# nickmass/mass-raytrace

Measured on AMD Instinct MI355X. Metric: Msamples/sec (rays traced/sec) at 1920×1080×1024spp; 1/2/4/8-GPU scaling, higher is better.
Workload: dtype f32

## Files before the change

mass-raytrace_amd/csrc/device/layout.h:

```cpp
#pragma once
#include <stdint.h>

#include "nf_bound.h"

namespace mrt {

enum : uint32_t { KIND_BOX = 1, KIND_SPHERE = 2, KIND_TRI = 3, KIND_INST = 4, KIND_MODEL = 5, KIND_VOLUME = 6 };
constexpr uint32_t kBoxFlag = 0x80000000u;
constexpr uint32_t kLdsTag = 0x40000000u;
constexpr uint32_t kIdxMask = 0x3FFFFFFFu;
constexpr uint32_t KIND_END = 0;
enum : uint32_t { TRI_FLAG_ALPHA = 1u, TRI_FLAG_UV = 2u, TRI_FLAG_EVE = 4u };
constexpr uint32_t kTriAlpha = 0x80000000u;
constexpr uint32_t kTriIdMask = 0x0FFFFFFFu;

constexpr uint32_t kNfIdx = 0x0FFFFFFFu;
constexpr uint32_t kNfForceL = 0x10000000u, kNfForceR = 0x20000000u;
constexpr uint32_t kNfPop = 0x0FFFFFFFu;
constexpr int kNfExpMin = -100;
constexpr uint32_t kNfStack = 24u;
constexpr uint32_t kNfWildFew = 16u;
constexpr uint32_t kNoParent = 0xFFFFFFFFu;
constexpr uint32_t kWorldKey = 0x80000000u;
enum : uint32_t { VNF_SPHERE = 0, VNF_TRI = 1, VNF_INST = 2, VNF_MODEL = 3 };

constexpr uint32_t SURF_PROGRAM = 0xFFu;
constexpr uint32_t kSurfStack = 4;
struct GpuSurfOp {
  uint32_t op, tex, arg, pad;
  float color[4];
};
struct GpuSurfRef {
  uint32_t kind, index, len, pad;
  float color[4];
};

struct GpuMaterial {
  uint32_t kind, surf_kind, texture;
  float param;
  float color[4];
  uint32_t left, right;
  uint32_t surf_len;
  uint32_t pad1;
// ... 23 lines not shown
  const uint32_t* sph_mat;
  const float* tri_shade;
  const GpuMaterial* materials;
  const GpuTexture* textures;
  const uint32_t* texels;
  uint32_t fast_ok;
  uint32_t n_slots, n_tris, n_sph, n_inst, n_models, n_materials, n_textures, n_texels;
  uint32_t* dbg;
  const float* vol_nid;
  const uint32_t* vol_mat;
  const float* ln_table;
  uint32_t n_vol;
  const GpuSurfOp* surf_ops;
  uint32_t n_surf_ops;
  uint32_t bg_kind;
  float bg_color[4];
  const GpuSurfRef* bg_faces;
  const float* bg_m;
  const uint32_t* slots_tl;
  const uint32_t* tlet;
  uint32_t n_tlet;
  uint32_t tl_world_begin;
  uint32_t nf_ok, nf_world;
  const uint32_t* vnf_leaf;
  uint32_t vnf_base[4];
  uint32_t n_vnf;
  NfBound nfb;
  const float* eve;
  const float* tri_tb;
  uint32_t n_eve;
};

}
```

mass-raytrace_amd/csrc/device/nf_tree.cpp:

```cpp
#include <math.h>
#include <cmath>
#include <string.h>

#include <algorithm>
#include <unordered_map>

#include "upload.h"

namespace mrt {

namespace {

float u2f(uint32_t u) {
  float f;
  memcpy(&f, &u, 4);
  return f;
}
uint32_t f2u(float f) {
  uint32_t u;
  memcpy(&u, &f, 4);
  return u;
}

uint32_t kind_of(const std::vector<uint32_t>& w, uint32_t i) { return w[4 * (i + 1) + 3]; }
// ... 593 lines not shown
    if (!ref_order(s.world_begin, true, world_objs)) return true;
    if (world_objs.empty()) return (s.nf_note = "an empty world", true);
    std::vector<std::vector<uint32_t>> blas_objs(s.blas_regions.size());
    if (s.keep_nf_boxes) {
      s.nf_leaf_box.assign(3 * s.vnf_leaf.size(), NAN);
      s.nf_inst_wild.assign(d.n_instances, 0);
    }
    for (size_t k = 0; k < s.blas_regions.size(); ++k) {
      region_of[s.blas_regions[k].begin] = k;
      if (!ref_order(s.blas_regions[k].begin, false, blas_objs[k])) return true;
    }
    std::vector<uint8_t> by_model(s.blas_regions.size(), 0), by_inst(s.blas_regions.size(), 0);
    for (uint32_t r : world_objs) {
      const uint32_t kd = kind_of(w, r);
      if (kd != KIND_INST && kd != KIND_MODEL) continue;
      auto it = region_of.find(w[4 * (size_t)r + 1]);
      if (it != region_of.end()) (kd == KIND_MODEL ? by_model : by_inst)[it->second] = 1;
    }
    const uint32_t has_blas = s.blas_regions.empty() ? 0 : 2;
    std::vector<Tree> blas(s.blas_regions.size());
    blas_box.assign(s.blas_regions.size(), Box{});
    blas_bound.assign(s.blas_regions.size(), TriBound{});
    uint32_t blas_depth = 0;
    const uint32_t world_min = Tree::min_levels((uint32_t)world_objs.size());
    if (world_min + has_blas > kNfStack) return (s.nf_note = "too many world objects for the walk's stack", true);
    for (size_t k = 0; k < blas.size(); ++k) {
      for (uint32_t r : blas_objs[k]) {
        blas[k].items.push_back({object_box(r, &blas_bound[k]), r});
        keep_box(r, blas[k].items.back().b);
      }
      if (blas[k].items.empty()) continue;
      blas[k].max_depth = kNfStack - 2 - world_min;
      blas[k].build(0, (uint32_t)blas[k].items.size(), 0);
      blas_depth = std::max(blas_depth, blas[k].depth);
      blas_box[k] = blas[k].nodes[0].b;
      if (by_model[k]) grow_bound(world_tri, blas_bound[k]);
    }
    Tree world;
    NfBound& B = s.nfb;
    B = NfBound{};
    double aw0 = 0, aw1 = 0, bw0 = 0, bw1 = 0, ko1 = 0, ao0 = 0, ao1 = 0, orad = 0;
    std::vector<Item> wild_items, items;
    Box gen_box;
    uint32_t n_world_inst = 0;
    for (uint32_t r : world_objs) n_world_inst += kind_of(w, r) == KIND_INST;
    const bool few = n_world_inst <= kNfWildFew;
    for (uint32_t r : world_objs) {
// ... 21 lines not shown
        ko1 = std::max(ko1, m.ko);
        if (it != region_of.end()) {
          const Box& bb = blas_box[it->second];
          for (int c = 0; c < 8; ++c) {
            const double x = c & 1 ? bb.mx[0] : bb.mn[0], y = c & 2 ? bb.mx[1] : bb.mn[1], z = c & 4 ? bb.mx[2] : bb.mn[2];
            orad = std::max(orad, std::sqrt(x * x + y * y + z * z));
          }
          ao0 = std::max(ao0, ob.a0), ao1 = std::max(ao1, ob.a1);
        }
        if (wild(m) || (few && m.b0 > 0x1p-14)) {
          wild_items.push_back({b, r, true});
          wild_term[r] = {b, m};
          s.nf_wild++;
          if (s.keep_nf_boxes) s.nf_inst_wild[w[4 * (size_t)r]] = 1;
          continue;
        }
        aw0 = std::max(aw0, m.w0), aw1 = std::max(aw1, m.w1), bw0 = std::max(bw0, m.b0), bw1 = std::max(bw1, m.b1);
      }
      if (generic) gen_box.grow(b);
      items.push_back({b, r});
    }
    aw0 = std::max(aw0, world_tri.a0), aw1 = std::max(aw1, world_tri.a1);
    if (r_min < 0x1p-60) return (s.nf_note = "a sphere too small for the walk's rounding bound", true);
    world.items = items;
    world.items.insert(world.items.end(), wild_items.begin(), wild_items.end());
    world.max_depth = kNfStack - (has_blas ? 2 + blas_depth : 0);
    world.build(0, (uint32_t)world.items.size(), 0);
    if (!wild_items.empty()) world.mark_forced(0);
    if (aw1 > 0 || ao1 > 0)
      for (Tree* t : [&] {
             std::vector<Tree*> v{&world};
             for (Tree& b : blas) v.push_back(&b);
             return v;
           }())
        fit_cones(*t);
    s.nf_stack_need = world.depth + (has_blas ? 2 + blas_depth : 0);
    if (s.nf_stack_need > kNfStack) return (s.nf_note = "trees deeper than the walk's stack", true);
    auto ball = [](const Box& b, float c[3], float& rr) {
      double r2 = 0;
      for (int k = 0; k < 3; ++k) {
        const double m = 0.5 * ((double)b.mn[k] + (double)b.mx[k]);
        c[k] = (float)m;
        const double e = std::max(std::fabs((double)b.mx[k] - c[k]), std::fabs(c[k] - (double)b.mn[k]));
        r2 += e * e;
      }
      rr = f_up(std::sqrt(r2) * (1 + 0x1p-40));
    };
    Box wb;
    for (const Item& it : items) wb.grow(it.b);
    if (items.empty()) wb = world.nodes[0].b;
    for (int k = 0; k < 3; ++k)
      if (!(std::fabs(wb.mn[k]) < INFINITY && std::fabs(wb.mx[k]) < INFINITY))
        return (s.nf_note = "a box the node format cannot hold (not finite)", true);
    ball(wb, B.wc, B.wr);
    if (aw1 > 0) ball(gen_box, B.gc, B.gr);
    B.aw0 = f_up(aw0), B.aw1 = f_up(aw1), B.bw0 = f_up(bw0 + 0x1p-90), B.bw1 = f_up(bw1);
    B.kw1 = f_up(world_tri.k1), B.ko1 = f_up(ko1);
    B.ao0 = f_up(ao0), B.ao1 = f_up(ao1), B.orad = f_up(orad);
    B.kmax = kNfKappaMax;
    B.kc = (aw1 > 0 || ao1 > 0) ? f_up(1.0001 * 24.0 * kU * 64.0 / (1.0 - 1.01 * (double)kNfKappaMax) * (1.0 + 0x1p-17))
                                : 0.0f;
    B.kcmin = 0.0f;
    if (!gen_extent.empty()) {
      std::nth_element(gen_extent.begin(), gen_extent.begin() + gen_extent.size() / 2, gen_extent.end());
      B.kcmin = std::ldexp(gen_extent[gen_extent.size() / 2], -6);
    }
    if (r_max > 0) {
      ball(sph_box, B.sc, B.sr);
      B.s51 = f_up(51.2 * kU / r_min), B.s28 = f_up(27.8 * kU), B.s130 = f_up(130.2 * kU), B.s11 = f_up(11.2 * kU * r_max);
    } else {
      B.sr = -1.0f;
    }
    s.nf_world = emit(world);
    if (s.nf_world == ~0u) return (s.nf_note = "a box the node format cannot hold (not finite)", true);
    for (size_t k = 0; k < blas.size(); ++k) {
      if (blas[k].items.empty()) continue;
      const uint32_t root = emit(blas[k]);
      if (root == ~0u) return (s.nf_note = "a box the node format cannot hold (not finite)", true);
      blas_root[s.blas_regions[k].begin] = root;
    }
    for (auto& [at, r] : wild_at) {
      const auto& [b, m] = wild_term.at(r);
      bool finite = true;
      for (int k = 0; k < 3; ++k) finite = finite && std::fabs(b.mn[k]) < INFINITY && std::fabs(b.mx[k]) < INFINITY;
      if (!finite) continue;
      float c[3], rr;
      ball(b, c, rr);
      const uint32_t e = push(f2u(b.mn[0]), f2u(b.mn[1]), f2u(b.mn[2]), f2u(b.mx[0]));
      push(f2u(b.mx[1]), f2u(b.mx[2]), f2u(f_up(m.w0)), f2u(f_up(m.w1)));
      push(f2u(f_up(m.b0 + 0x1p-90)), f2u(f_up(m.b1)), f2u(c[0]), f2u(c[1]));
      push(f2u(c[2]), f2u(rr), 0, 0);
      w[4 * (size_t)at + 3] = e;
    }
    for (auto& [rec, ref_blas] : patches) {
      auto it = blas_root.find(ref_blas);
      if (it == blas_root.end()) return (s.nf_note = "an instance of an empty BLAS", true);
      w[4 * rec + 1] = it->second;
    }
    if (n_slots() > kNfIdx) return (s.nf_note = "record stream past 2^28 slots", true);
    s.nf_ok = true;
    return true;
  }
};

}

bool build_nf_trees(const mrt_scene_desc& d, HostScene& s, std::string& err) {
  Builder b{d, s, err, s.slots, {}, {}};
  const size_t keep = s.slots.size();
  const bool ok = b.run();
  if (!s.nf_ok) {
    s.slots.resize(keep);
    s.nf_boxes = 0;
    s.nf_wild = 0;
    s.nf_cones = 0;
    s.vnf_leaf.clear();
  }
  return ok;
}

}
```

mass-raytrace_amd/csrc/device/trace.hip:

```cpp
#include <string.h>

#include <algorithm>

#include "ctx.h"

using namespace mrt;

namespace {

constexpr size_t kTraceLdsMaxBytes = 160 * 1024;
constexpr uint32_t kStashQuads = 4;

template <bool COUNT, bool LDS, uint32_t ALPHA, bool RNG, int BLK, bool NF = false>
__global__ __launch_bounds__(BLK) __attribute__((amdgpu_waves_per_eu(NF ? (COUNT ? 1 : 5) : (ALPHA == 0 && !RNG && !COUNT ? 8 : 1)))) void k_trace(DevScene S, PathBufs in, uint4* hits, Ctrl* ctrl, uint32_t cur,
                                                  DevCounters* cnt, float tmin, float tmax, TraceTune tune) {
  static_assert(!NF || (!LDS && !RNG), "the near-first walk has no treelet and no traversal draws");
  constexpr int R = 1;
  const uint32_t n = ctrl->active[cur];
  if (blockIdx.x == 0 && threadIdx.x == 0) {
    ctrl->active[cur ^ 1] = 0;
    ctrl->surv[cur ^ 1] = 0;
  }
  if (n == 0) return;
  if (LDS) {
    for (uint32_t k = threadIdx.x; k < S.n_tlet; k += BLK) mrt_lds[k] = reinterpret_cast<const uint4*>(S.tlet)[k];
    __syncthreads();
  }
  TravIn tin_{S, reinterpret_cast<const uint4*>(LDS ? S.slots_tl : S.slots), LDS ? S.tl_world_begin : S.world_begin,
              in.ro, in.rd, tmin, in.rng, tmax};
  if (!LDS && !NF) {
    tin_.stash = reinterpret_cast<float4*>(mrt_lds) + threadIdx.x;
    tin_.stash_stride = (uint32_t)BLK;
  }
  const TravIn& tin = tin_;
  const NfStack stk{reinterpret_cast<uint32_t*>(mrt_lds) + threadIdx.x, (uint32_t)BLK};
  LocalCounters lc;
  uint32_t seg = 0, nh = 0;
  uint32_t pool = 0, pool_end = 0;
  bool drained = false;
// ... 15 lines not shown
    }
    if (n_idle >= tune.refill * R || n_idle == 64u * R) {
      while (pool == pool_end && !drained) {
        const uint32_t lo = (uint32_t)((uint64_t)n * grp / kGroups), hi = (uint32_t)((uint64_t)n * (grp + 1) / kGroups);
        uint32_t b = 0;
        if (lane_id() == 0) b = atomicAdd(&ctrl->group_next[grp * 32], tune.chunk);
        b = __shfl(b, 0, 64);
        if (b < hi - lo) {
          pool = lo + b;
          pool_end = hi - pool > tune.chunk ? pool + tune.chunk : hi;
        } else if (++visited == kGroups) {
          drained = true;
        } else {
          grp = (grp + 1) % kGroups;
        }
      }
      const uint32_t avail = pool_end - pool;
      uint32_t off = 0;
      unsigned long long live = 0;
#pragma unroll
      for (int q = 0; q < R; ++q) {
        if (t[q].ray == kIdle) {
          const uint32_t r = off + lane_rank(idle[q]);
          if (r < avail) trav_init<RNG, LDS>(tin, t[q], MRT_IDX(S, pool + r, n, 20), tmax, NF ? S.nf_world : 0xFFFFFFFFu);
        }
        off += (uint32_t)__popcll(idle[q]);
        live |= __ballot(t[q].ray != kIdle);
      }
      pool += n_idle < avail ? n_idle : avail;
      if (live == 0) break;
    }
#pragma unroll
    for (int q = 0; q < R; ++q) {
      auto box_step = [&]() {
        const bool run_box = trav_at_box(t[q]);
        const unsigned long long bm = __builtin_amdgcn_ballot_w64(run_box);
        if ((uint32_t)__popcll(bm) < tune.box_min) return false;
        if (run_box) {
          if (NF && t[q].sp != kExactMode)
            trav_box_index_nf<COUNT>(tin, stk, t[q], lc);
          else
            trav_box_index<COUNT>(tin, t[q], lc);
        }
        if (run_box && (!NF || t[q].sp != kNfDone)) trav_fetch<LDS>(tin, t[q]);
        if (COUNT) {
          lc.wave_slots += lane_id() == 0 ? 64u : 0u;
          lc.lane_steps += run_box ? 1u : 0u;
        }
        return true;
      };
      while (box_step() && box_step()) {
      }
      for (;;) {
        const bool busy = !t[q].done && (!NF || t[q].sp != kNfDone);
        const bool at_box = busy && trav_at_box(t[q]);
        const unsigned long long box_mask = __ballot(at_box);
        const unsigned long long prim_mask = __ballot(busy && !at_box);
        const bool prim_run = NF && (uint32_t)__popcll(prim_mask) >= tune.prim_run;
        const bool box_go = at_box && !prim_run;
        const bool prim_go = (__popcll(prim_mask) >= tune.prim_batch || box_mask == 0) && busy && !at_box;
        if (box_go) {
          if (NF && t[q].sp != kExactMode)
            trav_box_index_nf<COUNT>(tin, stk, t[q], lc);
          else
            trav_box_index<COUNT>(tin, t[q], lc);
        }
        if (prim_go) {
          if (NF && t[q].sp != kExactMode)
            trav_prim_index_nf<COUNT, ALPHA>(tin, stk, t[q], lc);
          else
            trav_prim_index<COUNT, ALPHA, RNG, LDS>(tin, t[q], lc);
        }
        if ((box_go || prim_go) && !t[q].done && (!NF || t[q].sp != kNfDone)) trav_fetch<LDS>(tin, t[q]);
        if (COUNT) {
          lc.wave_slots += lane_id() == 0 ? 64u : 0u;
          lc.lane_steps += (box_go || prim_go) ? 1u : 0u;
        }
        if (!prim_run) break;
      }
      if (NF) {
        const bool over = t[q].sp == kNfDone;
        const unsigned long long om = __builtin_amdgcn_ballot_w64(over);
        if (om != 0 && ((uint32_t)__popcll(om) >= tune.nf_batch ||
                        __builtin_amdgcn_ballot_w64(!t[q].done && !over) == 0) && over) {
          nf_finish<COUNT>(tin, t[q], lc);
          if (!t[q].done) trav_fetch<LDS>(tin, t[q]);
        }
      }
    }
#pragma unroll
    for (int q = 0; q < R; ++q) {
      if (t[q].ray != kIdle && t[q].done) {
        if (RNG) trav_store_rng(tin, t[q]);
        const Hit h = trav_hit<LDS>(tin, t[q]);
        hits[t[q].ray] = make_uint4(__float_as_uint(h.t), h.prim, h.container, 0u);
        seg += 1;
        nh += t[q].prim != kRefNone;
        t[q].ray = kIdle;
      }
    }
  }
  if (COUNT) flush_counters(cnt, lc, seg, nh, 0, 0);
}
// ... 39 lines not shown
template <bool EXT>
__global__ __launch_bounds__(kBlock) void k_rays_out(DevScene S, PathBufs in, const uint4* hits, uint32_t n,
                                                     uint4* out) {
  uint32_t i = blockIdx.x * kBlock + threadIdx.x;
  if (i >= n) return;
  const float4 o4 = in.ro[i], d4 = in.rd[i];
  const uint4 hv = hits[i];
  Hit h{__uint_as_float(hv.x), hv.y, hv.z};
  uint32_t front = 0;
  LocalCounters lc;
  if (h.prim != kRefNone)
    front = resolve_hit<EXT>(S, V3{o4.x, o4.y, o4.z}, V3{d4.x, d4.y, d4.z}, h, lc).front_face ? 1u : 0u;
  out[i] = make_uint4(h.prim, h.container, __float_as_uint(h.prim != kRefNone ? h.t : 0.0f), front);
}

using TraceFn = void (*)(DevScene, PathBufs, uint4*, Ctrl*, uint32_t, DevCounters*, float, float, TraceTune);
template <bool COUNT, uint32_t ALPHA, bool RNG>
TraceFn trace_kernel_lds(int block) {
  return block == 1024  ? k_trace<COUNT, true, ALPHA, RNG, 1024>
         : block == 512 ? k_trace<COUNT, true, ALPHA, RNG, 512>
                        : k_trace<COUNT, true, ALPHA, RNG, kBlock>;
}
template <bool COUNT, uint32_t ALPHA>
TraceFn trace_kernel_a(bool lds, bool rng, int block, bool nf) {
  if (nf) return k_trace<COUNT, false, ALPHA, false, kBlock, true>;
  if (lds) return rng ? trace_kernel_lds<COUNT, ALPHA, true>(block) : trace_kernel_lds<COUNT, ALPHA, false>(block);
  return rng ? k_trace<COUNT, false, ALPHA, true, kBlock> : k_trace<COUNT, false, ALPHA, false, kBlock>;
}
template <bool COUNT>
TraceFn trace_kernel_c(bool lds, uint32_t alpha, bool rng, int block, bool nf) {
  return alpha == 2   ? trace_kernel_a<COUNT, 2>(lds, rng, block, nf)
         : alpha == 1 ? trace_kernel_a<COUNT, 1>(lds, rng, block, nf)
                      : trace_kernel_a<COUNT, 0>(lds, rng, block, nf);
}
TraceFn trace_kernel(bool count, bool lds, uint32_t alpha, bool rng, int block, bool nf) {
  return count ? trace_kernel_c<true>(lds, alpha, rng, block, nf) : trace_kernel_c<false>(lds, alpha, rng, block, nf);
}

}

uint32_t persistent_grid(mrt_ctx* c, const void* f, size_t smem, bool shared, int block, int share_num,
                         int share_den) {
  auto key = std::make_pair(f, smem);
  auto it = c->grids.find(key);
  if (it != c->grids.end()) return it->second;
  if (smem > 0) HIP_CHECK(hipFuncSetAttribute(f, hipFuncAttributeMaxDynamicSharedMemorySize, (int)kTraceLdsMaxBytes));
  int per_cu = 0;
  HIP_CHECK(hipOccupancyMaxActiveBlocksPerMultiprocessor(&per_cu, f, block, smem));
  if (shared) per_cu = std::max(1, per_cu * share_num / share_den);
  if (c->tun.wgs_per_cu) per_cu = (int)c->tun.wgs_per_cu;
  const uint32_t g = (uint32_t)c->cus * (uint32_t)std::max(1, per_cu);
  c->grids[key] = g;
  return g;
}

void launch_trace(mrt_ctx* c, hipStream_t st, const Queue& q, const PathBufs& in, uint32_t cur, bool count,
                  float tmin, float tmax) {
  const Tuning& t = c->tun;
  const bool nf = t.use_nf, lds = !nf && c->facts.treelet;
  const uint32_t alpha = c->scene_alpha ? (c->scene_ext ? 2u : 1u) : 0u;
  const int block = lds ? t.trace_block : kBlock;
  const TraceFn f = trace_kernel(count, lds, alpha, c->facts.trav_rng, block, nf);
  const size_t smem = nf ? (size_t)kNfStack * block * 4 : lds ? (size_t)c->S.n_tlet * 16 : (size_t)kStashQuads * block * 16;
  uint32_t grid = persistent_grid(c, (const void*)f, smem, t.queues > 1, block, nf ? 1 : 3, nf ? 1 : 4);
  const uint32_t nf_cap = 3u * (uint32_t)c->cus;
  if (nf && t.queues > 1 && !t.wgs_per_cu && grid > nf_cap) grid = c->grids[std::make_pair((const void*)f, smem)] = nf_cap;
  hipLaunchKernelGGL(f, dim3(grid), dim3(block), smem, st, c->S, in, q.hits, q.ctrl, cur, c->d_cnt, tmin, tmax, t.trace);
  HIP_CHECK(hipGetLastError());
}

void launch_trace_simple(mrt_ctx* c, const Queue& q, uint32_t cur) {
  auto* f = c->facts.trav_rng ? k_trace_simple<true> : k_trace_simple<false>;
  hipLaunchKernelGGL(f, dim3(c->trace_grid), dim3(kBlock), 0, q.stream, c->S, q.bufs[cur], q.hits, q.ctrl, cur, c->d_cnt);
  HIP_CHECK(hipGetLastError());
}

extern "C" int mrt_trace_rays(mrt_ctx* c, const float* rays, uint32_t n, float t_min, float t_max, mrt_hit* out) {
  MRT_DEV0(c, mrt_trace_rays(c, rays, n, t_min, t_max, out));
  return guarded(c, [&] {
    if (!c->has_scene) throw ApiError{MRT_ERR_STATE, "no scene uploaded"};
    if (n == 0) return;
    if (!rays || !out) throw ApiError{MRT_ERR_INVALID, "null argument"};
    if (n > c->rays_cap) {
      hipFree(c->d_rays);
      hipFree(c->d_rhits);
      c->d_rays = nullptr;
// ... 30 lines not shown
```

mass-raytrace_amd/csrc/device/upload.h:

```cpp
#pragma once
#include <string>
#include <vector>

#include "../../../include/massrt.h"
#include "layout.h"

namespace mrt {

struct BlasRegion {
  uint32_t begin, end, refs;
  bool model;
};

struct HostScene {
  std::vector<uint32_t> slots;
  std::vector<uint32_t> rec_starts;
  uint32_t world_begin = 0, world_end = 0;
  std::vector<float> inst_inv, inst_fwd;
  std::vector<uint32_t> inst_mat, model_mat;
  std::vector<float> sph;
  std::vector<uint32_t> sph_mat;
  std::vector<float> tri_shade;
  std::vector<float> eve;
  std::vector<float> tri_tb;
// ... 3 lines not shown
  uint32_t fast_ok = 1;
  uint32_t early_ok = 1;
  bool has_alpha = false;
  bool trav_rng = false;
  std::vector<float> vol_nid;
  std::vector<uint32_t> vol_mat;
  std::vector<float> ln_table;
  std::vector<GpuSurfOp> surf_ops;
  uint32_t bg_kind = 0;
  float bg_color[4] = {0, 0, 0, 0};
  std::vector<GpuSurfRef> bg_faces;
  float bg_m[16] = {0};
  std::vector<BlasRegion> blas_regions;
  std::vector<uint32_t> tlet, slots_tl;
  uint32_t tl_world_begin = 0, tl_boxes = 0;
  uint32_t n_box_records = 0, n_prim_records = 0, max_depth = 0;
  bool nf_ok = false;
  uint32_t nf_world = 0, nf_boxes = 0, nf_stack_need = 0, nf_first_slot = 0;
  std::vector<uint32_t> vnf_leaf;
  uint32_t vnf_base[4] = {0, 0, 0, 0};
  std::string nf_note;
  NfBound nfb{};
  uint32_t nf_wild = 0;
  uint32_t nf_cones = 0;
  bool keep_nf_boxes = false;
  int nf_build = 2;
  std::vector<float> nf_leaf_box;
  std::vector<uint8_t> nf_inst_wild;
};

enum { kNfBuildNever = 0, kNfBuildAlways = 1, kNfBuildAuto = 2 };

inline DevScene host_dev_scene(const HostScene& s) {
  DevScene S{};
  S.slots = s.slots.data();
  S.world_begin = s.world_begin;
  S.world_end = s.world_end;
  S.inst_inv = s.inst_inv.data();
  S.inst_fwd = s.inst_fwd.data();
  S.inst_mat = s.inst_mat.data();
  S.model_mat = s.model_mat.data();
  S.sph = s.sph.data();
  S.sph_mat = s.sph_mat.data();
  S.tri_shade = s.tri_shade.data();
  S.materials = s.materials.data();
  S.textures = s.textures.data();
  S.texels = s.texels.data();
  S.fast_ok = (s.fast_ok ? 1u : 0u) | (s.early_ok ? 2u : 0u);
  S.n_slots = (uint32_t)(s.slots.size() / 4);
  S.n_tris = (uint32_t)(s.tri_shade.size() / (kTriShadeQuads * 4));
  S.n_sph = (uint32_t)s.sph_mat.size();
  S.n_inst = (uint32_t)s.inst_mat.size();
  S.n_models = (uint32_t)s.model_mat.size();
  S.n_materials = (uint32_t)s.materials.size();
  S.n_textures = (uint32_t)s.textures.size();
  S.n_texels = (uint32_t)s.texels.size();
  S.vol_nid = s.vol_nid.data();
  S.vol_mat = s.vol_mat.data();
  S.ln_table = s.ln_table.empty() ? nullptr : s.ln_table.data();
  S.n_vol = (uint32_t)s.vol_nid.size();
  S.surf_ops = s.surf_ops.data();
  S.n_surf_ops = (uint32_t)s.surf_ops.size();
  S.bg_kind = s.bg_kind;
  for (int k = 0; k < 4; ++k) S.bg_color[k] = s.bg_color[k];
  S.bg_faces = s.bg_faces.data();
  S.bg_m = s.bg_m;
  S.nf_ok = s.nf_ok ? 1u : 0u;
  S.nf_world = s.nf_world;
  S.vnf_leaf = s.vnf_leaf.data();
  for (int k = 0; k < 4; ++k) S.vnf_base[k] = s.vnf_base[k];
  S.n_vnf = (uint32_t)(s.vnf_leaf.size() / 2);
  S.nfb = s.nfb;
  S.eve = s.eve.data();
  S.tri_tb = s.tri_tb.empty() ? nullptr : s.tri_tb.data();
  S.n_eve = (uint32_t)(s.eve.size() / (kEveQuads * 4));
  return S;
}

bool build_nf_trees(const mrt_scene_desc& d, HostScene& s, std::string& err);

bool build_host_scene(const mrt_scene_desc& d, HostScene& out, std::string& err, bool sibling_layout = true,
                      const mrt_scene_ext* ext = nullptr);

void build_treelet(HostScene& s, uint32_t budget);

}
```

mass-raytrace_amd/csrc/device/walk.h:

```cpp
#pragma once
#include "isect.h"

namespace mrt {

struct Hit {
  float t;
  uint32_t prim;
  uint32_t container;
};

struct TravIn {
  const DevScene& S;
  const uint4* slots;
  uint32_t world_begin;
  const float4* ro;
  const float4* rd;
  float tmin;
  uint4* rng = nullptr;
  float tmax0 = INFINITY;
  float4* stash = nullptr;
  uint32_t stash_stride = 0;
};
MRT_HD void tray_stash(const TravIn& in, const TRay& r) {
  float4* p = in.stash;
  const uint32_t k = in.stash_stride;
  p[0] = make_float4(r.o.x, r.o.y, r.o.z, r.d.x);
  p[k] = make_float4(r.d.y, r.d.z, r.yx, r.yy);
  p[2 * k] = make_float4(r.yz, r.oyx, r.oyy, r.oyz);
  p[3 * k] = make_float4(r.om, r.a.b, r.a.y, 0.0f);
}
MRT_HD TRay tray_unstash(const TravIn& in) {
  const float4* p = in.stash;
  const uint32_t k = in.stash_stride;
  const float4 a = p[0], b = p[k], c = p[2 * k], e = p[3 * k];
  TRay r;
  r.o = V3{a.x, a.y, a.z};
  r.d = V3{a.w, b.x, b.y};
  r.yx = b.z, r.yy = b.w, r.yz = c.x;
  r.oyx = c.y, r.oyy = c.z, r.oyz = c.w;
  r.om = e.x;
  r.a.b = e.y, r.a.y = e.z;
  return r;
}

constexpr uint32_t kNoRet = 0xFFFFFFFFu;
constexpr uint32_t kRetInstance = 0x80000000u;
constexpr uint32_t kExactMode = 0xFFFFu;

struct Trav {
  TRay r;
  uint32_t ray;
  uint32_t i, ret;
  float best;
  uint32_t prim, hit_ret;
  uint4 s0, s1;
  PathRng rng;
  uint32_t sp;
  float t2;
  NfLine nfl;
  float nl;
  bool done;
#ifdef MRT_DEBUG_BOUNDS
  uint32_t steps;
#endif
};

extern __shared__ uint4 mrt_lds[];
template <bool LDS>
MRT_HD void rec_load2(const TravIn& in, uint32_t i, uint4& a, uint4& b) {
#if defined(__HIP_DEVICE_COMPILE__)
// ... 43 lines not shown
    return;
  }
#endif
  rec_load2<LDS>(in, t.i, t.s0, t.s1);
}

MRT_HD void trav_end_index(const TravIn& in, Trav& t) {
  if (t.ret == kNoRet) {
    t.done = true;
    return;
  }
  if (t.ret & kRetInstance) t.r = in.stash ? tray_unstash(in) : world_ray(in, t.ray);
  t.i = t.ret & ~kRetInstance;
  t.ret = kNoRet;
}

MRT_HD float nf_cull(float best) { return fmaf(fabsf(best), 0x1p-10f, best); }
MRT_HD void nf_margin(const TravIn& in, Trav& t) {
  const bool obj = t.ret != kNoRet && (t.ret & kRetInstance);
  const NfBound& B = in.S.nfb;
  const NfCoef c = obj ? nf_coef_object(B, t.r.o, t.r.a.b) : nf_coef_world(B, t.r.o, t.r.a.b);
  t.nfl = nf_line(B, c, nf_cull(t.best), obj ? B.ao0 : B.aw0, obj ? B.ao1 : B.aw1, t.r.a.b, t.r.d);
}
MRT_HD void nf_start(const TravIn& in, Trav& t) {
  if (nf_ray_ok(in.S.nfb, t.r.a.b)) {
    nf_margin(in, t);
    t.nl = INFINITY;
  } else {
    t.i = in.world_begin;
    t.sp = kExactMode;
  }
}

template <bool RNG = false, bool LDS = false>
MRT_HD void trav_init(const TravIn& in, Trav& t, uint32_t ray, float tmax, uint32_t start = 0xFFFFFFFFu) {
  if (RNG) {
    const uint4 q = in.rng[ray];
    t.rng = PathRng{(unsigned long long)q.x | ((unsigned long long)q.y << 32),
                    (unsigned long long)q.z | ((unsigned long long)q.w << 32)};
  }
  t.r = world_ray(in, ray);
  t.ray = ray;
  t.i = start == 0xFFFFFFFFu ? in.world_begin : start;
  t.sp = start == 0xFFFFFFFFu ? kExactMode : 0u;
  t.t2 = INFINITY;
  t.ret = kNoRet;
  t.best = tmax;
  t.prim = kRefNone;
  t.hit_ret = kNoRet;
  t.done = false;
#ifdef MRT_DEBUG_BOUNDS
  t.steps = 0;
#endif
  if (start != 0xFFFFFFFFu) nf_start(in, t);
  trav_fetch<LDS>(in, t);
}

MRT_HD bool trav_at_box(const Trav& t) { return (int32_t)t.s1.w < 0; }

template <bool COUNT>
MRT_HD void trav_box_index(const TravIn& in, Trav& t, LocalCounters& lc) {
  if (COUNT) lc.node_visits++;
  V3 mn{u2f(t.s0.x), u2f(t.s0.y), u2f(t.s0.z)}, mx{u2f(t.s0.w), u2f(t.s1.x), u2f(t.s1.y)};
  t.i = box_hit_any<COUNT>(mn, mx, t.r, in.tmin, t.best, &lc) ? (t.s1.w & ~kBoxFlag) : t.s1.z;
}
template <bool COUNT, bool LDS = false>
MRT_HD void trav_box(const TravIn& in, Trav& t, LocalCounters& lc) {
  trav_box_index<COUNT>(in, t, lc);
  trav_fetch<LDS>(in, t);
}

MRT_HD void trav_store_rng(const TravIn& in, const Trav& t) {
  in.rng[t.ray] = make_uint4((uint32_t)t.rng.s0, (uint32_t)(t.rng.s0 >> 32), (uint32_t)t.rng.s1,
                             (uint32_t)(t.rng.s1 >> 32));
}

MRT_HD bool volume_hit(const DevScene& S, const TravIn& in, Trav& t, uint4 s0, uint32_t vid, float& th) {
  const V3 c{u2f(s0.x), u2f(s0.y), u2f(s0.z)};
// ... 94 lines not shown
```

mass-raytrace_amd/csrc/device/walk_nf.h:

```cpp
#pragma once
#include "walk.h"

namespace mrt {

constexpr uint32_t kNfDone = 0xFFFEu;
constexpr uint32_t kNfRet = 0x80000000u;

struct NfStack {
  uint32_t* p;
  uint32_t stride;
};
MRT_HD void nf_push(const NfStack& k, Trav& t, uint32_t v) {
  k.p[t.sp * k.stride] = v;
  t.sp += 1;
}
MRT_HD bool nf_pop(const TravIn& in, const NfStack& k, Trav& t) {
  if (t.sp == 0) return false;
  t.sp -= 1;
  t.nl = INFINITY;
  uint32_t v = k.p[t.sp * k.stride];
  if (v == kNfRet) {
    const bool inst = (t.ret & kRetInstance) != 0;
    t.ret = kNoRet;
    if (inst) {
      t.r = world_ray(in, t.ray);
      nf_margin(in, t);
    }
    if (t.sp == 0) return false;
    t.sp -= 1;
    v = k.p[t.sp * k.stride];
  }
  t.i = v;
  return true;
}
MRT_HD uint32_t vnf_entry(const DevScene& S, uint32_t base, uint32_t id, uint32_t word) {
  return S.vnf_leaf[2 * (size_t)MRT_IDX(S, S.vnf_base[base] + id, S.n_vnf, 23) + word];
}
MRT_HD unsigned long long nf_key(const TravIn& in, uint32_t prim, uint32_t ret) {
  const DevScene& S = in.S;
  const uint32_t kind = prim >> 28, id = prim & 0x0FFFFFFFu;
  if (kind == MRT_REF_SPHERE) return (unsigned long long)vnf_entry(S, VNF_SPHERE, id, 1) << 32;
  const uint32_t k = vnf_entry(S, VNF_TRI, id, 1);
  if (k & kWorldKey) return (unsigned long long)(k & ~kWorldKey) << 32;
  const uint32_t rec = (ret & ~kRetInstance) - 2;
  const uint32_t cid = in.slots[MRT_IDX(S, rec, S.n_slots, 24)].x;
  const uint32_t wk = vnf_entry(S, (ret & kRetInstance) ? VNF_INST : VNF_MODEL, cid, 1);
  return ((unsigned long long)wk << 32) | k;
}
MRT_HD bool nf_better(const TravIn& in, const Trav& t, float th, uint32_t prim) {
  if (th < t.best) return true;
  if (!(th == t.best)) return false;
  if (t.prim == kRefNone) return true;
  return nf_key(in, prim, t.ret) > nf_key(in, t.prim, t.hit_ret);
}
MRT_HD void nf_hit(const TravIn& in, Trav& t, float th, uint32_t prim) {
  bool better = th < t.best;
// ... 105 lines not shown
      const float t1 = vmin3(vmax1(a.x, bb.x), vmax1(a.y, bb.y), vmin1(vmax1(a.z, bb.z), tmax));
      dt[c] = t0[c] - t1;
      m[c] = 0.0f;
      xb[c] = INFINITY;
    }
  }
#pragma unroll
  for (int c = 0; c < 2; ++c) {
    const bool force = (s1.w & (kNfForceL << c)) != 0;
    hit[c] = !(dt[c] > m[c]) || force;
    ent[c] = t0[c];
    ex[c] = force ? INFINITY : xb[c];
  }
}

MRT_HD bool wave_any(bool p) {
#if defined(__HIP_DEVICE_COMPILE__)
  return __builtin_amdgcn_ballot_w64(p) != 0;
#else
  return p;
#endif
}

template <bool COUNT>
MRT_HD void trav_box_index_nf(const TravIn& in, const NfStack& k, Trav& t, LocalCounters& lc) {
  if (COUNT) lc.node_visits += 2;
  bool h[2];
  float e[2], x[2];
  const float cb = nf_cull(t.best);
#ifdef MRT_PROBE_NF_ZERO_RHO
  const float rho = 0.0f;
#elif defined(MRT_PROBE_NF_NOCONE)
  const float rho = nf_rho_node(t.nfl, fminf(cb, t.nl));
#else
  const float tn = vmin1(cb, t.nl);
  float rho = nf_rho_node(t.nfl, tn);
  if (in.S.nfb.kc > 0.0f && wave_any(t.nfl.rg * tn > in.S.nfb.kcmin))
    rho = nf_rho_cone(t.nfl, tn, t.s0.x, t.s0.y, t.s0.z, t.s0.w, t.r.d);
#endif
  nf_node_test(t.s0, t.s1, t.r, in.tmin, cb, rho, h, e, x);
  const uint32_t base = t.s1.w & kNfIdx, right = base + 2u + ((t.s0.w >> 24) & 1u);
  const bool left = h[0] && (!h[1] || !(e[1] < e[0]));
  t.i = left ? base : right;
  t.nl = left ? x[0] : x[1];
  if (h[0] && h[1]) nf_push(k, t, left ? right : base);
  if (!(h[0] || h[1]) && !nf_pop(in, k, t)) nf_over(t);
}

MRT_HD bool nf_wild_enter(const TravIn& in, const Trav& t, uint32_t at) {
  const uint4 a = rec_load1<false>(in, at), b = rec_load1<false>(in, at + 1), c = rec_load1<false>(in, at + 2),
              e = rec_load1<false>(in, at + 3);
  const NfWild x{{u2f(a.x), u2f(a.y), u2f(a.z)}, {u2f(a.w), u2f(b.x), u2f(b.y)}, u2f(b.z), u2f(b.w), u2f(c.x), u2f(c.y),
                 {u2f(c.z), u2f(c.w), u2f(e.x)}, u2f(e.y)};
  return nf_wild_hit(x, t.r.o, t.r.d, t.r.a.b, in.tmin, nf_cull(t.best));
}

template <bool COUNT, uint32_t ALPHA>
MRT_HD void trav_prim_index_nf(const TravIn& in, const NfStack& k, Trav& t, LocalCounters& lc) {
  const DevScene& S = in.S;
  const uint4 s0 = t.s0, s1 = t.s1;
  const uint32_t kind = s1.w;
  uint32_t next;
  if (kind == KIND_TRI) {
    if (COUNT) lc.triangle_tests++;
    const uint4 s2 = rec_load1<false>(in, t.i + 2);
    V3 a{u2f(s0.x), u2f(s0.y), u2f(s0.z)}, ab{u2f(s0.w), u2f(s1.x), u2f(s1.y)}, ac{u2f(s2.x), u2f(s2.y), u2f(s2.z)};
    float th;
    if (tri_hit_nb(a, ab, ac, t.r.o, t.r.d, in.tmin, nf_cull(t.best), th)) {
      const uint32_t id = s1.z & kTriIdMask;
      if (!ALPHA || !(s1.z & kTriAlpha) || tri_alpha_pass<false, ALPHA == 2>(S, id, t.r.o, t.r.d, th, t.rng, lc))
        nf_hit(in, t, th, make_ref(MRT_REF_TRIANGLE, id));
    }
    next = s2.w;
  } else if (kind == KIND_SPHERE) {
    if (COUNT) lc.sphere_tests++;
    float th;
    if (sphere_hit(V3{u2f(s0.x), u2f(s0.y), u2f(s0.z)}, u2f(s0.w), t.r.o, t.r.d, t.r.a, in.tmin, nf_cull(t.best), th))
      nf_hit(in, t, th, make_ref(MRT_REF_SPHERE, s1.x));
    next = s1.y;
  } else if (kind == KIND_INST && s0.w != 0 && !nf_wild_enter(in, t, s0.w)) {
    next = s0.z;
  } else {
    if (s0.z != kNfPop) nf_push(k, t, s0.z);
    nf_push(k, t, kNfRet);
    if (kind == KIND_INST) {
      if (COUNT) lc.instance_entries++;
      V3 c0, c1, c2, c3;
      load_m12(S.inst_inv + (size_t)MRT_IDX(S, s0.x, S.n_inst, 8) * 12, c0, c1, c2, c3);
      t.r = make_tray(xform(c0, c1, c2, c3, t.r.o, 1.0f), xform(c0, c1, c2, c3, t.r.d, 0.0f), S.fast_ok);
      t.ret = (t.i + 2) | kRetInstance;
      nf_margin(in, t);
    } else {
      if (COUNT) lc.model_entries++;
      t.ret = t.i + 2;
    }
    t.i = s0.y;
    return;
  }
  t.i = next;
  if (next == kNfPop && !nf_pop(in, k, t)) nf_over(t);
}

}
```

Measured before the change: 1287.

## Split wild instances into a separate tree walked after the regular world tree

When wild (forced-entry) instances exist and the world has no model objects, they are built into their own BVH instead of being mixed into the world tree. The world root is then no longer force-marked. Each ray pushes a marker on its stack and parks in a wait state when it reaches that marker. Waiting lanes are batched across the wave and resumed at the wild tree root, so ordinary rays get tighter culling in the world tree. This costs one extra stack slot, a new wave-level batching step, and sentinel renumbering (kExactMode, kNfDone, kNfWait).

```diff
diff --git a/mass-raytrace_amd/csrc/device/layout.h b/mass-raytrace_amd/csrc/device/layout.h
--- a/mass-raytrace_amd/csrc/device/layout.h
+++ b/mass-raytrace_amd/csrc/device/layout.h
@@ -18,7 +18,7 @@
 constexpr uint32_t kNfForceL = 0x10000000u, kNfForceR = 0x20000000u;
 constexpr uint32_t kNfPop = 0x0FFFFFFFu;
 constexpr int kNfExpMin = -100;
-constexpr uint32_t kNfStack = 24u;
+constexpr uint32_t kNfStack = 25u;
 constexpr uint32_t kNfWildFew = 16u;
 constexpr uint32_t kNoParent = 0xFFFFFFFFu;
 constexpr uint32_t kWorldKey = 0x80000000u;
@@ -88,6 +88,7 @@
   uint32_t n_tlet;
   uint32_t tl_world_begin;
   uint32_t nf_ok, nf_world;
+  uint32_t nf_wild_root;
   const uint32_t* vnf_leaf;
   uint32_t vnf_base[4];
   uint32_t n_vnf;
diff --git a/mass-raytrace_amd/csrc/device/nf_tree.cpp b/mass-raytrace_amd/csrc/device/nf_tree.cpp
--- a/mass-raytrace_amd/csrc/device/nf_tree.cpp
+++ b/mass-raytrace_amd/csrc/device/nf_tree.cpp
@@ -639,7 +639,7 @@
     blas_box.assign(s.blas_regions.size(), Box{});
     blas_bound.assign(s.blas_regions.size(), TriBound{});
     uint32_t blas_depth = 0;
-    const uint32_t world_min = Tree::min_levels((uint32_t)world_objs.size());
+    const uint32_t world_min = Tree::min_levels((uint32_t)world_objs.size()) + 1;
     if (world_min + has_blas > kNfStack) return (s.nf_note = "too many world objects for the walk's stack", true);
     for (size_t k = 0; k < blas.size(); ++k) {
       for (uint32_t r : blas_objs[k]) {
@@ -707,20 +707,33 @@
     }
     aw0 = std::max(aw0, world_tri.a0), aw1 = std::max(aw1, world_tri.a1);
     if (r_min < 0x1p-60) return (s.nf_note = "a sphere too small for the walk's rounding bound", true);
+    Tree wild_tree;
+    bool has_model = false;
+    for (const Item& it : items) has_model = has_model || kind_of(w, it.rec) == KIND_MODEL;
+    const bool split = !wild_items.empty() && !items.empty() && !has_model;
+    const uint32_t below = has_blas ? 2 + blas_depth : 0;
     world.items = items;
-    world.items.insert(world.items.end(), wild_items.begin(), wild_items.end());
-    world.max_depth = kNfStack - (has_blas ? 2 + blas_depth : 0);
+    if (!split) world.items.insert(world.items.end(), wild_items.begin(), wild_items.end());
+    world.max_depth = kNfStack - below - 1;
     world.build(0, (uint32_t)world.items.size(), 0);
-    if (!wild_items.empty()) world.mark_forced(0);
+    if (split) {
+      wild_tree.items = wild_items;
+      wild_tree.max_depth = kNfStack - below;
+      wild_tree.build(0, (uint32_t)wild_tree.items.size(), 0);
+      wild_tree.mark_forced(0);
+    } else if (!wild_items.empty()) {
+      world.mark_forced(0);
+    }
     if (aw1 > 0 || ao1 > 0)
       for (Tree* t : [&] {
              std::vector<Tree*> v{&world};
+             if (split) v.push_back(&wild_tree);
              for (Tree& b : blas) v.push_back(&b);
              return v;
            }())
         fit_cones(*t);
-    s.nf_stack_need = world.depth + (has_blas ? 2 + blas_depth : 0);
-    if (s.nf_stack_need > kNfStack) return (s.nf_note = "trees deeper than the walk's stack", true);
+    s.nf_stack_need = std::max(world.depth + (split ? 1u : 0u), wild_tree.depth) + below;
+    if (s.nf_stack_need > kNfStack - (split ? 0u : 1u)) return (s.nf_note = "trees deeper than the walk's stack", true);
     auto ball = [](const Box& b, float c[3], float& rr) {
       double r2 = 0;
       for (int k = 0; k < 3; ++k) {
@@ -758,6 +771,11 @@
     }
     s.nf_world = emit(world);
     if (s.nf_world == ~0u) return (s.nf_note = "a box the node format cannot hold (not finite)", true);
+    s.nf_wild_root = 0;
+    if (split) {
+      s.nf_wild_root = emit(wild_tree);
+      if (s.nf_wild_root == ~0u) return (s.nf_note = "a box the node format cannot hold (not finite)", true);
+    }
     for (size_t k = 0; k < blas.size(); ++k) {
       if (blas[k].items.empty()) continue;
       const uint32_t root = emit(blas[k]);
@@ -798,6 +816,7 @@
     s.slots.resize(keep);
     s.nf_boxes = 0;
     s.nf_wild = 0;
+    s.nf_wild_root = 0;
     s.nf_cones = 0;
     s.vnf_leaf.clear();
   }
diff --git a/mass-raytrace_amd/csrc/device/trace.hip b/mass-raytrace_amd/csrc/device/trace.hip
--- a/mass-raytrace_amd/csrc/device/trace.hip
+++ b/mass-raytrace_amd/csrc/device/trace.hip
@@ -11,10 +11,11 @@
 constexpr size_t kTraceLdsMaxBytes = 160 * 1024;
 constexpr uint32_t kStashQuads = 4;
 
-template <bool COUNT, bool LDS, uint32_t ALPHA, bool RNG, int BLK, bool NF = false>
+template <bool COUNT, bool LDS, uint32_t ALPHA, bool RNG, int BLK, bool NF = false, bool WILD = false>
 __global__ __launch_bounds__(BLK) __attribute__((amdgpu_waves_per_eu(NF ? (COUNT ? 1 : 5) : (ALPHA == 0 && !RNG && !COUNT ? 8 : 1)))) void k_trace(DevScene S, PathBufs in, uint4* hits, Ctrl* ctrl, uint32_t cur,
                                                   DevCounters* cnt, float tmin, float tmax, TraceTune tune) {
   static_assert(!NF || (!LDS && !RNG), "the near-first walk has no treelet and no traversal draws");
+  static_assert(!WILD || NF, "only the near-first walk has a wild tree");
   constexpr int R = 1;
   const uint32_t n = ctrl->active[cur];
   if (blockIdx.x == 0 && threadIdx.x == 0) {
@@ -76,7 +77,12 @@
       for (int q = 0; q < R; ++q) {
         if (t[q].ray == kIdle) {
           const uint32_t r = off + lane_rank(idle[q]);
-          if (r < avail) trav_init<RNG, LDS>(tin, t[q], MRT_IDX(S, pool + r, n, 20), tmax, NF ? S.nf_world : 0xFFFFFFFFu);
+          if (r < avail) {
+            if constexpr (NF)
+              trav_init_nf<WILD>(tin, stk, t[q], MRT_IDX(S, pool + r, n, 20), tmax, S.nf_world);
+            else
+              trav_init<RNG, LDS>(tin, t[q], MRT_IDX(S, pool + r, n, 20), tmax);
+          }
         }
         off += (uint32_t)__popcll(idle[q]);
         live |= __ballot(t[q].ray != kIdle);
@@ -92,11 +98,11 @@
         if ((uint32_t)__popcll(bm) < tune.box_min) return false;
         if (run_box) {
           if (NF && t[q].sp != kExactMode)
-            trav_box_index_nf<COUNT>(tin, stk, t[q], lc);
+            trav_box_index_nf<COUNT, WILD>(tin, stk, t[q], lc);
           else
             trav_box_index<COUNT>(tin, t[q], lc);
         }
-        if (run_box && (!NF || t[q].sp != kNfDone)) trav_fetch<LDS>(tin, t[q]);
+        if (run_box && (!NF || !nf_parked<WILD>(t[q]))) trav_fetch<LDS>(tin, t[q]);
         if (COUNT) {
           lc.wave_slots += lane_id() == 0 ? 64u : 0u;
           lc.lane_steps += run_box ? 1u : 0u;
@@ -106,7 +112,7 @@
       while (box_step() && box_step()) {
       }
       for (;;) {
-        const bool busy = !t[q].done && (!NF || t[q].sp != kNfDone);
+        const bool busy = !t[q].done && (!NF || !nf_parked<WILD>(t[q]));
         const bool at_box = busy && trav_at_box(t[q]);
         const unsigned long long box_mask = __ballot(at_box);
         const unsigned long long prim_mask = __ballot(busy && !at_box);
@@ -115,17 +121,17 @@
         const bool prim_go = (__popcll(prim_mask) >= tune.prim_batch || box_mask == 0) && busy && !at_box;
         if (box_go) {
           if (NF && t[q].sp != kExactMode)
-            trav_box_index_nf<COUNT>(tin, stk, t[q], lc);
+            trav_box_index_nf<COUNT, WILD>(tin, stk, t[q], lc);
           else
             trav_box_index<COUNT>(tin, t[q], lc);
         }
         if (prim_go) {
           if (NF && t[q].sp != kExactMode)
-            trav_prim_index_nf<COUNT, ALPHA>(tin, stk, t[q], lc);
+            trav_prim_index_nf<COUNT, ALPHA, WILD>(tin, stk, t[q], lc);
           else
             trav_prim_index<COUNT, ALPHA, RNG, LDS>(tin, t[q], lc);
         }
-        if ((box_go || prim_go) && !t[q].done && (!NF || t[q].sp != kNfDone)) trav_fetch<LDS>(tin, t[q]);
+        if ((box_go || prim_go) && !t[q].done && (!NF || !nf_parked<WILD>(t[q]))) trav_fetch<LDS>(tin, t[q]);
         if (COUNT) {
           lc.wave_slots += lane_id() == 0 ? 64u : 0u;
           lc.lane_steps += (box_go || prim_go) ? 1u : 0u;
@@ -133,6 +139,15 @@
         if (!prim_run) break;
       }
       if (NF) {
+        if (WILD) {
+          const bool wait = t[q].sp == kNfWait;
+          const unsigned long long wm = __builtin_amdgcn_ballot_w64(wait);
+          if (wm != 0 && ((uint32_t)__popcll(wm) >= tune.nf_batch ||
+                          __builtin_amdgcn_ballot_w64(!t[q].done && !nf_parked<WILD>(t[q])) == 0) && wait) {
+            nf_resume_wild(tin, t[q]);
+            trav_fetch<LDS>(tin, t[q]);
+          }
+        }
         const bool over = t[q].sp == kNfDone;
         const unsigned long long om = __builtin_amdgcn_ballot_w64(over);
         if (om != 0 && ((uint32_t)__popcll(om) >= tune.nf_batch ||
@@ -218,19 +233,19 @@
                         : k_trace<COUNT, true, ALPHA, RNG, kBlock>;
 }
 template <bool COUNT, uint32_t ALPHA>
-TraceFn trace_kernel_a(bool lds, bool rng, int block, bool nf) {
-  if (nf) return k_trace<COUNT, false, ALPHA, false, kBlock, true>;
+TraceFn trace_kernel_a(bool lds, bool rng, int block, bool nf, bool wild) {
+  if (nf) return wild ? k_trace<COUNT, false, ALPHA, false, kBlock, true, true> : k_trace<COUNT, false, ALPHA, false, kBlock, true, false>;
   if (lds) return rng ? trace_kernel_lds<COUNT, ALPHA, true>(block) : trace_kernel_lds<COUNT, ALPHA, false>(block);
   return rng ? k_trace<COUNT, false, ALPHA, true, kBlock> : k_trace<COUNT, false, ALPHA, false, kBlock>;
 }
 template <bool COUNT>
-TraceFn trace_kernel_c(bool lds, uint32_t alpha, bool rng, int block, bool nf) {
-  return alpha == 2   ? trace_kernel_a<COUNT, 2>(lds, rng, block, nf)
-         : alpha == 1 ? trace_kernel_a<COUNT, 1>(lds, rng, block, nf)
-                      : trace_kernel_a<COUNT, 0>(lds, rng, block, nf);
-}
-TraceFn trace_kernel(bool count, bool lds, uint32_t alpha, bool rng, int block, bool nf) {
-  return count ? trace_kernel_c<true>(lds, alpha, rng, block, nf) : trace_kernel_c<false>(lds, alpha, rng, block, nf);
+TraceFn trace_kernel_c(bool lds, uint32_t alpha, bool rng, int block, bool nf, bool wild) {
+  return alpha == 2   ? trace_kernel_a<COUNT, 2>(lds, rng, block, nf, wild)
+         : alpha == 1 ? trace_kernel_a<COUNT, 1>(lds, rng, block, nf, wild)
+                      : trace_kernel_a<COUNT, 0>(lds, rng, block, nf, wild);
+}
+TraceFn trace_kernel(bool count, bool lds, uint32_t alpha, bool rng, int block, bool nf, bool wild) {
+  return count ? trace_kernel_c<true>(lds, alpha, rng, block, nf, wild) : trace_kernel_c<false>(lds, alpha, rng, block, nf, wild);
 }
 
 }
@@ -256,8 +271,9 @@
   const bool nf = t.use_nf, lds = !nf && c->facts.treelet;
   const uint32_t alpha = c->scene_alpha ? (c->scene_ext ? 2u : 1u) : 0u;
   const int block = lds ? t.trace_block : kBlock;
-  const TraceFn f = trace_kernel(count, lds, alpha, c->facts.trav_rng, block, nf);
-  const size_t smem = nf ? (size_t)kNfStack * block * 4 : lds ? (size_t)c->S.n_tlet * 16 : (size_t)kStashQuads * block * 16;
+  const bool wild = nf && c->S.nf_wild_root != 0;
+  const TraceFn f = trace_kernel(count, lds, alpha, c->facts.trav_rng, block, nf, wild);
+  const size_t smem = nf ? (size_t)(kNfStack - (wild ? 0u : 1u)) * block * 4 : lds ? (size_t)c->S.n_tlet * 16 : (size_t)kStashQuads * block * 16;
   uint32_t grid = persistent_grid(c, (const void*)f, smem, t.queues > 1, block, nf ? 1 : 3, nf ? 1 : 4);
   const uint32_t nf_cap = 3u * (uint32_t)c->cus;
   if (nf && t.queues > 1 && !t.wgs_per_cu && grid > nf_cap) grid = c->grids[std::make_pair((const void*)f, smem)] = nf_cap;
diff --git a/mass-raytrace_amd/csrc/device/upload.h b/mass-raytrace_amd/csrc/device/upload.h
--- a/mass-raytrace_amd/csrc/device/upload.h
+++ b/mass-raytrace_amd/csrc/device/upload.h
@@ -49,6 +49,7 @@
   std::string nf_note;
   NfBound nfb{};
   uint32_t nf_wild = 0;
+  uint32_t nf_wild_root = 0;
   uint32_t nf_cones = 0;
   bool keep_nf_boxes = false;
   int nf_build = 2;
@@ -94,6 +95,7 @@
   S.bg_m = s.bg_m;
   S.nf_ok = s.nf_ok ? 1u : 0u;
   S.nf_world = s.nf_world;
+  S.nf_wild_root = s.nf_ok ? s.nf_wild_root : 0u;
   S.vnf_leaf = s.vnf_leaf.data();
   for (int k = 0; k < 4; ++k) S.vnf_base[k] = s.vnf_base[k];
   S.n_vnf = (uint32_t)(s.vnf_leaf.size() / 2);
diff --git a/mass-raytrace_amd/csrc/device/walk.h b/mass-raytrace_amd/csrc/device/walk.h
--- a/mass-raytrace_amd/csrc/device/walk.h
+++ b/mass-raytrace_amd/csrc/device/walk.h
@@ -45,7 +45,7 @@
 
 constexpr uint32_t kNoRet = 0xFFFFFFFFu;
 constexpr uint32_t kRetInstance = 0x80000000u;
-constexpr uint32_t kExactMode = 0xFFFFu;
+constexpr uint32_t kExactMode = 0xFFFDu;
 
 struct Trav {
   TRay r;
@@ -135,8 +135,29 @@
   const NfCoef c = obj ? nf_coef_object(B, t.r.o, t.r.a.b) : nf_coef_world(B, t.r.o, t.r.a.b);
   t.nfl = nf_line(B, c, nf_cull(t.best), obj ? B.ao0 : B.aw0, obj ? B.ao1 : B.aw1, t.r.a.b, t.r.d);
 }
-MRT_HD void nf_start(const TravIn& in, Trav& t) {
+constexpr uint32_t kNfWildMark = 0x80000001u;
+struct NfStack {
+  uint32_t* p;
+  uint32_t stride;
+};
+MRT_HD void nf_push(const NfStack& k, Trav& t, uint32_t v) {
+  k.p[t.sp * k.stride] = v;
+  t.sp += 1;
+}
+#if defined(__HIP_DEVICE_COMPILE__)
+#define MRT_PIN_VGPR(x) asm volatile("" : "+v"(x))
+#else
+#define MRT_PIN_VGPR(x) (void)0
+#endif
+template <bool WILD>
+MRT_HD void nf_start(const TravIn& in, const NfStack& k, Trav& t) {
   if (nf_ray_ok(in.S.nfb, t.r.a.b)) {
+    if (WILD) {
+      uint32_t mark = kNfWildMark;
+      MRT_PIN_VGPR(mark);
+      nf_push(k, t, mark);
+      MRT_PIN_VGPR(t.best);
+    }
     nf_margin(in, t);
     t.nl = INFINITY;
   } else {
@@ -145,8 +166,8 @@
   }
 }
 
-template <bool RNG = false, bool LDS = false>
-MRT_HD void trav_init(const TravIn& in, Trav& t, uint32_t ray, float tmax, uint32_t start = 0xFFFFFFFFu) {
+template <bool RNG, bool LDS, bool NF, bool WILD>
+MRT_HD void trav_begin(const TravIn& in, const NfStack& stk, Trav& t, uint32_t ray, float tmax, uint32_t start) {
   if (RNG) {
     const uint4 q = in.rng[ray];
     t.rng = PathRng{(unsigned long long)q.x | ((unsigned long long)q.y << 32),
@@ -154,8 +175,8 @@
   }
   t.r = world_ray(in, ray);
   t.ray = ray;
-  t.i = start == 0xFFFFFFFFu ? in.world_begin : start;
-  t.sp = start == 0xFFFFFFFFu ? kExactMode : 0u;
+  t.i = NF ? start : in.world_begin;
+  t.sp = NF ? 0u : kExactMode;
   t.t2 = INFINITY;
   t.ret = kNoRet;
   t.best = tmax;
@@ -165,8 +186,16 @@
 #ifdef MRT_DEBUG_BOUNDS
   t.steps = 0;
 #endif
-  if (start != 0xFFFFFFFFu) nf_start(in, t);
+  if (NF) nf_start<WILD>(in, stk, t);
   trav_fetch<LDS>(in, t);
+}
+template <bool RNG = false, bool LDS = false>
+MRT_HD void trav_init(const TravIn& in, Trav& t, uint32_t ray, float tmax) {
+  trav_begin<RNG, LDS, false, false>(in, NfStack{nullptr, 0}, t, ray, tmax, 0u);
+}
+template <bool WILD>
+MRT_HD void trav_init_nf(const TravIn& in, const NfStack& stk, Trav& t, uint32_t ray, float tmax, uint32_t start) {
+  trav_begin<false, false, true, WILD>(in, stk, t, ray, tmax, start);
 }
 
 MRT_HD bool trav_at_box(const Trav& t) { return (int32_t)t.s1.w < 0; }
diff --git a/mass-raytrace_amd/csrc/device/walk_nf.h b/mass-raytrace_amd/csrc/device/walk_nf.h
--- a/mass-raytrace_amd/csrc/device/walk_nf.h
+++ b/mass-raytrace_amd/csrc/device/walk_nf.h
@@ -3,35 +3,42 @@
 
 namespace mrt {
 
-constexpr uint32_t kNfDone = 0xFFFEu;
+constexpr uint32_t kNfDone = 0xFFFFu;
 constexpr uint32_t kNfRet = 0x80000000u;
-
-struct NfStack {
-  uint32_t* p;
-  uint32_t stride;
-};
-MRT_HD void nf_push(const NfStack& k, Trav& t, uint32_t v) {
-  k.p[t.sp * k.stride] = v;
-  t.sp += 1;
-}
+constexpr uint32_t kNfWait = 0xFFFEu;
+template <bool WILD>
+MRT_HD bool nf_parked(const Trav& t) { return WILD ? t.sp >= kNfWait : t.sp == kNfDone; }
+
+template <bool WILD>
 MRT_HD bool nf_pop(const TravIn& in, const NfStack& k, Trav& t) {
   if (t.sp == 0) return false;
   t.sp -= 1;
   t.nl = INFINITY;
   uint32_t v = k.p[t.sp * k.stride];
-  if (v == kNfRet) {
-    const bool inst = (t.ret & kRetInstance) != 0;
-    t.ret = kNoRet;
-    if (inst) {
-      t.r = world_ray(in, t.ray);
-      nf_margin(in, t);
-    }
-    if (t.sp == 0) return false;
-    t.sp -= 1;
-    v = k.p[t.sp * k.stride];
+  if (WILD ? (int32_t)v < 0 : v == kNfRet) {
+    if (!WILD || v == kNfRet) {
+      const bool inst = (t.ret & kRetInstance) != 0;
+      t.ret = kNoRet;
+      if (inst) {
+        t.r = world_ray(in, t.ray);
+        nf_margin(in, t);
+      }
+      if (t.sp == 0) return false;
+      t.sp -= 1;
+      v = k.p[t.sp * k.stride];
+    }
+    if (WILD && v == kNfWildMark) {
+      t.sp = kNfWait;
+      t.s1.w = KIND_END;
+      return true;
+    }
   }
   t.i = v;
   return true;
+}
+MRT_HD void nf_resume_wild(const TravIn& in, Trav& t) {
+  t.sp = 0;
+  t.i = in.S.nf_wild_root;
 }
 MRT_HD uint32_t vnf_entry(const DevScene& S, uint32_t base, uint32_t id, uint32_t word) {
   return S.vnf_leaf[2 * (size_t)MRT_IDX(S, S.vnf_base[base] + id, S.n_vnf, 23) + word];
@@ -183,7 +190,7 @@
 #endif
 }
 
-template <bool COUNT>
+template <bool COUNT, bool WILD>
 MRT_HD void trav_box_index_nf(const TravIn& in, const NfStack& k, Trav& t, LocalCounters& lc) {
   if (COUNT) lc.node_visits += 2;
   bool h[2];
@@ -205,7 +212,7 @@
   t.i = left ? base : right;
   t.nl = left ? x[0] : x[1];
   if (h[0] && h[1]) nf_push(k, t, left ? right : base);
-  if (!(h[0] || h[1]) && !nf_pop(in, k, t)) nf_over(t);
+  if (!(h[0] || h[1]) && !nf_pop<WILD>(in, k, t)) nf_over(t);
 }
 
 MRT_HD bool nf_wild_enter(const TravIn& in, const Trav& t, uint32_t at) {
@@ -216,7 +223,7 @@
   return nf_wild_hit(x, t.r.o, t.r.d, t.r.a.b, in.tmin, nf_cull(t.best));
 }
 
-template <bool COUNT, uint32_t ALPHA>
+template <bool COUNT, uint32_t ALPHA, bool WILD>
 MRT_HD void trav_prim_index_nf(const TravIn& in, const NfStack& k, Trav& t, LocalCounters& lc) {
   const DevScene& S = in.S;
   const uint4 s0 = t.s0, s1 = t.s1;
@@ -259,7 +266,7 @@
     return;
   }
   t.i = next;
-  if (next == kNfPop && !nf_pop(in, k, t)) nf_over(t);
-}
-
-}
+  if (next == kNfPop && !nf_pop<WILD>(in, k, t)) nf_over(t);
+}
+
+}
```

Result: faster. 1318 (median of 6 runs) (+2.4%).
